# OpenSpaceAI/Nesie

Hardware: AMD Instinct MI355X
Metric: ScanNet scenes/sec (fwd+bwd, 40k pts, bs=8) (higher is better)
Workload: dtype f32; 1 GPU; Nesie-VoteNet supervised pretrain step (nesie-votenet-scannet-pretrain-10%): fwd+bwd+AdamW, 40000 pts/scene, fp32, random-init weights; scenes_per_gpu=8, global_batch=8, parallelism=single, world_size=1, hip_graph=True, deterministic_backward=True, index_chain_pipelined=True, forward_cu_budget=232, forward_cu_budget_from_the_head_on=248, grad_allreduce_bytes=10561936, resident_input_scenes=0

## Files before the change

### include/nesie_ops.h

```cpp
#ifndef NESIE_OPS_H_
#define NESIE_OPS_H_

#include <stddef.h>
#include <stdint.h>

#ifdef __cplusplus
extern "C" {
#endif

typedef enum {
  NESIE_OK = 0,
  NESIE_ERR_INVALID_ARG = 1,
  NESIE_ERR_UNSUPPORTED = 2,
  NESIE_ERR_LAUNCH = 3
} nesie_status;

int nesie_abi_version(void);
const char *nesie_last_error(void);

int nesie_set_distance_form(int form);
int nesie_get_distance_form(void);
int nesie_set_cu_count(int n);
int nesie_get_cu_count(void);

// ... 260 lines not shown

int nesie_pool_tail_pack(int nb, int c, int m, const float *grad_pooled, const float *pooled,
                         const uint8_t *argmax, float *ent, void *stream);
int nesie_pw_dgrad_bn_reduce_sparse(int nb, int ng, int c, int cout, long long p, int ns,
                                    const float *ent, const float *w, long long w_gstride,
                                    int w_rstride, int w_cstride, float *y, long long y_bstride,
                                    const float *bn_z, long long bnz_bstride, const float *bn_coef,
                                    float *bn_part, void *stream);
int nesie_pw_wgrad_sparse_supported(int co, int ci, long long p, int ns);
int nesie_pw_wgrad_sparse(int nb, int ng, int co, int ci, long long p, int ns, const float *ent,
                          const float *x, long long x_bstride, const float *x_coef, float *dw,
                          void *workspace, size_t workspace_bytes, int defer, void *stream);

int nesie_pw_wgrad_supported(int co, int ci, long long p);
int nesie_pw_wgrad_tiled(int nb, int ng, int co, int ci, long long p);
size_t nesie_pw_wgrad_workspace_bytes(int nb, int ng, int co, int ci, long long p);
int nesie_pw_wgrad(int nb, int ng, int co, int ci, long long p, const float *dy,
                   long long dy_bstride, const float *x, long long x_bstride,
                   const float *x_coef, int x_relu, float *dw, void *workspace,
                   size_t workspace_bytes, int defer, void *stream);

int nesie_pw_wgrad_flush_deferred(void *stream);
int nesie_pw_wgrad_pending(void);
int nesie_pw_wgrad_drop_deferred(void);

int nesie_pw_wgrad_bn_supported(int co, int ci, long long p);
int nesie_pw_wgrad_bn_backward(int nb, int ng, int co, int ci, long long p, const float *da,
                               const float *z, long long z_bstride, const float *z_coef,
                               const float *gamma, const float *part, int nslots, const float *x,
                               long long x_bstride, const float *x_coef, int x_relu, float *dz,
                               float *dw, float *dgamma, float *dbeta, float *coef_ws,
                               float *d_row_bias, int rb_group, void *workspace,
                               size_t workspace_bytes, int defer, void *stream);

long long nesie_mlp_stream_partials(int b, long long p);
int nesie_mlp_stat_finalize(int c, long long nparts, double count, const float *stat_partial,
                            const float *gamma, const float *beta, float *running_mean,
                            float *running_var, float momentum, float eps, float *coef,
                            int channel_major, void *stream);
int nesie_mlp_layer_forward_stream(int b, int cin, int cout, long long p, const float *x,
                                   long long x_bstride, const float *w, const float *in_coef,
                                   int in_relu, float *y, float *stat_partial, void *stream);

int nesie_pw_layer_forward_k4(int nb, int cout, long long p, const float *x4, long long x4_bstride,
                              const float *w0, const float *w, int w_rstride, int w_cstride,
                              const float *in_coef, float *y, long long y_bstride, float *stat_part,
                              void *stream);
int nesie_pw_dgrad_bn_reduce_k4(int nb, int k, long long p, const float *x, long long x_bstride,
                                const float *w, int w_rstride, int w_cstride, const float *x4,
                                long long x4_bstride, const float *w0, const float *bn_coef,
                                float *bn_part, float *g_part, void *stream);
int nesie_pw_wgrad_bn_backward_k4(int nb, long long p, const float *da, const float *z,
                                  long long z_bstride, const float *z_coef, const float *gamma,
                                  const float *part, int nslots, const float *x4,
                                  long long x4_bstride, const float *w0, const float *x_coef,
                                  float *dz, float *dw, float *dgamma, float *dbeta, float *coef_ws,
                                  void *workspace, size_t workspace_bytes, int defer, void *stream);
int nesie_pw_wgrad_bn_backward_k4_slots(int nb, long long p);
int nesie_pw_wgrad_bn_backward_k4_fused(int nb, long long p, const float *da, const float *z,
                                        long long z_bstride, const float *z_coef, const float *gamma,
                                        const float *part, int nslots, const float *x4,
                                        long long x4_bstride, const float *w0, const float *x_coef,
                                        const float *w, float *dw, float *dgamma, float *dbeta,
                                        float *coef_ws, float *in_part, float *in_gpart,
                                        void *workspace, size_t workspace_bytes, int defer, void *stream);
size_t nesie_k4_moments_bytes(void);
// ... 23 lines not shown
```

### nesie_amd/csrc/pwconv_wgrad.hip

```cpp
#include "pwconv_fwd.h"

using namespace nesie;

namespace nesie {

template <int CO16, int CI16, int WM, int WN, bool AFF, bool BNB, bool K4 = false, bool FDG = false>
__global__ __launch_bounds__(512, FDG ? 4 : 1) void pw_wgrad_kernel(
    int nb, int ng, int co_all, int ci_all, long long p, const float *__restrict__ dy, long long dy_bs,
    const float *__restrict__ x, long long x_bs, const float *__restrict__ x_coef, int coef_gs,
    float x_lo, float *__restrict__ partial, int nwg_g, const float *__restrict__ bnz,
    const float *__restrict__ bnb, float *dz, float *__restrict__ d_rb, int rb_group, int rev,
    const float *__restrict__ k4_w, const float *__restrict__ fdg_w = nullptr, float *__restrict__ fdg_part = nullptr,
    float *__restrict__ fdg_gpart = nullptr) {
  const int row0 = blockIdx.y * CO16 * 16, col0 = blockIdx.z * CI16 * 16;
  const int co = co_all - row0 < CO16 * 16 ? co_all - row0 : CO16 * 16;
  const int ci = ci_all - col0 < CI16 * 16 ? ci_all - col0 : CI16 * 16;
  dy += (size_t)row0 * p;
  x += (size_t)col0 * p;
  if (AFF) x_coef += (size_t)col0 * 4;
  partial += (size_t)(blockIdx.y * gridDim.z + blockIdx.z) * ng * nwg_g * (CO16 * 16) * (CI16 * 16);
  constexpr int MB = CO16 / WM, NB = CI16 / WN, PT = 32, PITCH = PT + 4, CPR = PT / 4;
  constexpr int ROWS = (CO16 + CI16) * 16, NT = 512;
  constexpr int NX = (ROWS * CPR + NT - 1) / NT;
  constexpr bool EVEN = ROWS * CPR == NX * NT;
  constexpr int DYSLOTS = CO16 * 16 * CPR / NT;
  static_assert(WM * WN == 8 && CO16 % WM == 0 && CI16 % WN == 0 && (CO16 * 16 * CPR) % NT == 0, "tiling");
  extern __shared__ __attribute__((aligned(16))) float lds[];
  constexpr int TILE = ROWS * PITCH + (FDG ? 4 * PITCH : 0);
  static_assert(!FDG || (K4 && BNB && CO16 == 4 && CI16 == 4), "FDG: the 64 x 64 layer over a rebuilt operand");
  const int tid = threadIdx.x, lane = tid & 63, quad = lane >> 4, l16 = lane & 15;
  const int wave = __builtin_amdgcn_readfirstlane(tid >> 6);
  const int wm = wave / WN, wn = wave % WN;
  const int g = blockIdx.x % ng, rank = blockIdx.x / ng;

  static_assert(!K4 || (AFF && NX - DYSLOTS == 1 && CI16 == 4 && EVEN), "K4: one slot of X rows");
  float4 k4w = make_float4(0.f, 0.f, 0.f, 0.f);
  unsigned k4off = 0;
  bool k4row0 = false;
  f32x4 k4x[K4 ? 3 : 1];
  unsigned goff[NX], lw[NX];
  bool okslot[NX];
  float sc[AFF ? NX : 1], bi[AFF ? NX : 1];
  float zsc[BNB ? DYSLOTS : 1], zbi[BNB ? DYSLOTS : 1], za[BNB ? DYSLOTS : 1], zmu[BNB ? DYSLOTS : 1], zd1[BNB ? DYSLOTS : 1], ze0[BNB ? DYSLOTS : 1];
#pragma unroll
  for (int i = 0; i < NX; ++i) {
    const int c = i * NT + tid;
    const int row = c / CPR, cp = c % CPR;
    const bool isdy = i < DYSLOTS;
    const int r = isdy ? row : row - CO16 * 16;
    const bool ok = (EVEN || c < ROWS * CPR) && r < (isdy ? co : ci);
    okslot[i] = ok;
    goff[i] = ok ? (unsigned)(((size_t)r * p + cp * 4) * 4) : 0u;
    lw[i] = (unsigned)((row * PITCH + cp * 4) * 4);
    if constexpr (K4) {
      if (!isdy) {
        k4w = *(const float4 *)(k4_w + (size_t)r * 4);
        k4off = (unsigned)(cp * 16);
        k4row0 = r == 0;
        asm volatile("" : "+v"(k4w.x), "+v"(k4w.y), "+v"(k4w.z), "+v"(k4w.w));
      }
    }
    if (AFF) {
// ... 33 lines not shown
    const float *dyb = dy + pend, *xb = x + (size_t)n * x_bs + p0;
#pragma unroll
    for (int i = 0; i < NX; ++i) {
      unsigned o = goff[i];
      asm volatile("" : "+v"(o));
      if constexpr (K4) {
        if (i >= DYSLOTS) {
          unsigned o4 = k4off;
          asm volatile("" : "+v"(o4));
          stg[i] = load16_saddr(o4, xb);
#pragma unroll
          for (int j = 1; j < 4; ++j) k4x[j - 1] = load16_saddr(o4, xb + (size_t)j * p);
          continue;
        }
      }
      stg[i] = load16_saddr(o, i < DYSLOTS ? dyb : xb);
      if constexpr (BNB) {
        if (i < DYSLOTS) stz[i] = load16_saddr(o, bnz + pend);
      }
    }
  };
  auto write_tile = [&](float *buf) {
#pragma unroll
    for (int i = 0; i < NX; ++i) {
      f32x4 q = stg[i];
      if constexpr (BNB) {
        if (i < DYSLOTS) {
#pragma unroll
          for (int e = 0; e < 4; ++e) {
            const float zz = stz[i][e];
            const float gg = __builtin_fmaf(zz, zsc[i], zbi[i]) > 0.f ? q[e] : 0.f;
            q[e] = __builtin_fmaf(za[i], gg, __builtin_fmaf(zmu[i] - zz, zd1[i], ze0[i]));
          }
          if constexpr (!FDG) {
            if (pend_ok && okslot[i]) *(f32x4 *)((char *)(dz + pend) + goff[i]) = q;
          }
          if (d_rb) {
            float tsum = (q[0] + q[1]) + (q[2] + q[3]);
            tsum += __shfl_xor(tsum, 1, 64);
            tsum += __shfl_xor(tsum, 2, 64);
            if (rb_group == 64) tsum += __shfl_xor(tsum, 4, 64);
            const int c_ = i * NT + tid, row = c_ / CPR, cp = c_ % CPR;
            const bool writer = rb_group == 64 ? cp == 0 : (cp & 3) == 0;
            if (pend_ok && okslot[i] && writer) {
              const int gsh = rb_group == 64 ? 6 : 4;
              float *dst = d_rb + ((size_t)pend_n * co + row) * (size_t)(p >> gsh) + ((pend_p0 + 4 * cp) >> gsh);
              if (rb_group == 64) atomicAdd(dst, tsum); else *dst = tsum;
            }
          }
        }
      }
      if constexpr (K4) {
        if (i >= DYSLOTS) {
          if constexpr (FDG) {
            if (k4row0) {
              float *xt = buf + ROWS * PITCH + (k4off >> 2);
              *(f32x4 *)(xt) = q;
              *(f32x4 *)(xt + PITCH) = k4x[0];
              *(f32x4 *)(xt + 2 * PITCH) = k4x[1];
              *(f32x4 *)(xt + 3 * PITCH) = k4x[2];
            }
          }
#pragma unroll
          for (int e = 0; e < 4; ++e) q[e] = k4_dot(k4w, q[e], k4x[0][e], k4x[1][e], k4x[2][e]);
        }
      }
      if (AFF && i >= DYSLOTS) {
#pragma unroll
        for (int e = 0; e < 4; ++e) q[e] = fmaxf(__builtin_fmaf(q[e], sc[i], bi[i]), x_lo);
      }
      if (!(EVEN && all_rows)) q = okslot[i] ? q : (f32x4){0.f, 0.f, 0.f, 0.f};
      if (EVEN || (i * NT + tid) < ROWS * CPR) *(f32x4 *)((char *)buf + lw[i]) = q;
    }
  };

  f32x4 acc[MB][NB];
#pragma unroll
  for (int i = 0; i < MB; ++i)
#pragma unroll
    for (int j = 0; j < NB; ++j) acc[i][j] = (f32x4){0.f, 0.f, 0.f, 0.f};
  const int cb = wave & 3, ph = wave >> 2;
  float fw[FDG ? 16 : 1];
  float4 fw0 = make_float4(0.f, 0.f, 0.f, 0.f), fco = fw0;
  float fr0 = 0.f, fr1 = 0.f, fgx[4] = {0.f, 0.f, 0.f, 0.f};
  if constexpr (FDG) {
    const int c = 16 * cb + l16;
#pragma unroll
    for (int kk = 0; kk < 16; ++kk) fw[kk] = fdg_w[(size_t)(4 * kk + quad) * 64 + c];
    fw0 = *(const float4 *)(k4_w + (size_t)c * 4);
    fco = *(const float4 *)(x_coef + (size_t)c * 4);
#pragma unroll
    for (int kk = 0; kk < 16; ++kk) asm volatile("" : "+v"(fw[kk]));
    asm volatile("" : "+v"(fw0.x), "+v"(fw0.y), "+v"(fw0.z), "+v"(fw0.w), "+v"(fco.x), "+v"(fco.y), "+v"(fco.z), "+v"(fco.w));
  }

  float *b0 = lds, *b1 = lds + TILE;
  int t = rank;
  if (t < ntiles) {
    load_tile(t);
    write_tile(b0);
    load_tile(t + nwg_g);
  }
  for (; t < ntiles; t += nwg_g) {
    lgkm_wait<0>();
    __builtin_amdgcn_s_barrier();
    const unsigned la = lds_addr(b0) + (unsigned)(((wm * MB * 16 + l16) * PITCH + 4 * quad) * 4);
    const unsigned lb = lds_addr(b0) + (unsigned)(((CO16 * 16 + wn * NB * 16 + l16) * PITCH + 4 * quad) * 4);
    f32x4 fa[MB], fb[NB];
    static_for<0, 2>([&](auto pgc) {
      constexpr int pg = decltype(pgc)::value;
      static_for<0, MB>([&](auto ic) {
        constexpr int i = decltype(ic)::value;
        fa[i] = lds_read_b128<(i * 16 * PITCH + 16 * pg) * 4>(la);
      });
      static_for<0, NB>([&](auto jc) {
        constexpr int j = decltype(jc)::value;
        fb[j] = lds_read_b128<(j * 16 * PITCH + 16 * pg) * 4>(lb);
      });
      lgkm_wait<0>();
      __builtin_amdgcn_sched_barrier(0);
      static_for<0, 4>([&](auto cc) {
        constexpr int c = decltype(cc)::value;
        static_for<0, MB>([&](auto ic) {
          constexpr int i = decltype(ic)::value;
          static_for<0, NB>([&](auto jc) {
            constexpr int j = decltype(jc)::value;
            acc[i][j] = __builtin_amdgcn_mfma_f32_16x16x4f32(fa[i][c], fb[j][c], acc[i][j], 0, 0, 0);
          });
        });
      });
      __builtin_amdgcn_sched_barrier(0);
    });
    if constexpr (FDG) {
      f32x4 da = {0.f, 0.f, 0.f, 0.f};
      const float *az = b0 + quad * PITCH + 16 * ph + l16;
#pragma unroll
      for (int kk = 0; kk < 16; ++kk)
        da = __builtin_amdgcn_mfma_f32_16x16x4f32(az[kk * 4 * PITCH], fw[kk], da, 0, 0, 0);
      const float *xt = b0 + ROWS * PITCH + 16 * ph + 4 * quad;
      const f32x4 x0 = *(const f32x4 *)xt, x1 = *(const f32x4 *)(xt + PITCH), x2 = *(const f32x4 *)(xt + 2 * PITCH),
                  x3 = *(const f32x4 *)(xt + 3 * PITCH);
#pragma unroll
      for (int r = 0; r < 4; ++r) {
        const float z = k4_dot(fw0, x0[r], x1[r], x2[r], x3[r]);
        const float gg = __builtin_fmaf(z, fco.x, fco.y) > 0.f ? da[r] : 0.f;
        fr0 += gg;
        fr1 += gg * ((z - fco.z) * fco.w);
        fgx[0] = __builtin_fmaf(gg, x0[r], fgx[0]);
        fgx[1] = __builtin_fmaf(gg, x1[r], fgx[1]);
        fgx[2] = __builtin_fmaf(gg, x2[r], fgx[2]);
        fgx[3] = __builtin_fmaf(gg, x3[r], fgx[3]);
      }
    }
    write_tile(b1);
    __builtin_amdgcn_sched_barrier(0);
    load_tile(t + 2 * nwg_g);
    float *const tb = b0; b0 = b1; b1 = tb;
  }
  if constexpr (FDG) {
    float v[6] = {fr0, fr1, fgx[0], fgx[1], fgx[2], fgx[3]};
#pragma unroll
    for (int u = 0; u < 6; ++u) {
      v[u] += __shfl_xor(v[u], 16, 64);
      v[u] += __shfl_xor(v[u], 32, 64);
    }
    if (quad == 0) {
      const int c = 16 * cb + l16, slot = 2 * rank + ph, nslots = 2 * nwg_g;
      *(float2 *)(fdg_part + ((size_t)c * nslots + slot) * 2) = make_float2(v[0], v[1]);
      *(float4 *)(fdg_gpart + ((size_t)c * nslots + slot) * 4) = make_float4(v[2], v[3], v[4], v[5]);
    }
  }
  const bool tiled = gridDim.y * gridDim.z > 1;
  float *dst = partial + ((size_t)g * nwg_g + rank) * (tiled ? (size_t)(CO16 * 16) * (CI16 * 16) : (size_t)co * ci);
#pragma unroll
  for (int i = 0; i < MB; ++i)
#pragma unroll
    for (int j = 0; j < NB; ++j)
#pragma unroll
      for (int r = 0; r < 4; ++r) {
        const int m = (wm * MB + i) * 16 + 4 * quad + r, k = (wn * NB + j) * 16 + l16;
        if (m < co && k < ci) dst[(size_t)m * ci + k] = acc[i][j][r];
      }
}

__global__ __launch_bounds__(512) void pw_wgrad_sparse_kernel(int nb, int ng, long long p, const float *__restrict__ x,
                                                              long long x_bs, const float *__restrict__ coef,
                                                              const float2 *__restrict__ ent, int ns_shift,
                                                              int groups, float *__restrict__ partial, int nwg,
// ... 249 lines not shown
constexpr int TILED_B = 64, TILED_MAX_TILES = 1024;
static bool pw_wgrad_tiled(int nb, int ng, int co, int ci, long long p) {
  if (nb <= 0 || ng <= 0 || nb % ng || p <= 0 || p % 32 || ci < 9 || ci > 1024 || co < 1 || co > 1024) return false;
  const long long tiles = (long long)(nb / ng) * (p / 32);
  return tiles <= TILED_MAX_TILES && (long long)co * ci >= 128 * 192;
}
static int pw_wgrad_tiled_nwg(int nb, int ng, int co, int ci, long long p) {
  const long long tiles = (long long)(nb / ng) * (p / 32);
  const int blocks = cdiv(co, TILED_B) * cdiv(ci, TILED_B);
  long long nwg = 512 / ((long long)blocks * ng);
  if (nwg < 1) nwg = 1;
  if (nwg > tiles) nwg = tiles;
  return (int)nwg;
}

extern "C" int nesie_pw_wgrad_tiled(int nb, int ng, int co, int ci, long long p) {
  return pw_wgrad_tiled(nb, ng, co, ci, p) ? 1 : 0;
}

extern "C" size_t nesie_pw_wgrad_workspace_bytes(int nb, int ng, int co, int ci, long long p) {
  if (nb <= 0 || ng <= 0 || p <= 0) return 0;
  const size_t whole = (size_t)ng * pw_wgrad_nwg(nb, ng, p, co, pw_wgrad_block(co, ci)) * co * pw_wgrad_block(co, ci) * sizeof(float);
  const size_t tiled = (size_t)cdiv(co, TILED_B) * cdiv(ci, TILED_B) * ng * pw_wgrad_tiled_nwg(nb, ng, co, ci, p) *
                       TILED_B * TILED_B * sizeof(float);
  return whole > tiled ? whole : tiled;
}

namespace nesie {
__global__ __launch_bounds__(64) void pw_bnb_coef_kernel(int channels, int nslots, double count,
                                                         const float *__restrict__ part,
                                                         const float *__restrict__ z_coef,
                                                         const float *__restrict__ gamma,
                                                         float *__restrict__ bnb, float *__restrict__ dgamma,
                                                         float *__restrict__ dbeta) {
  const int c = blockIdx.x;
  double s0 = 0.0, s1 = 0.0;
  const float2 *pc = (const float2 *)part + (size_t)c * nslots;
  int i = threadIdx.x;
  for (; i + 192 < nslots; i += 256) {
    float2 q[4];
#pragma unroll
    for (int u = 0; u < 4; ++u) q[u] = pc[i + 64 * u];
#pragma unroll
    for (int u = 0; u < 4; ++u) { s0 += (double)q[u].x; s1 += (double)q[u].y; }
  }
  for (; i < nslots; i += 64) {
    const float2 q = pc[i];
    s0 += (double)q.x;
    s1 += (double)q.y;
  }
#pragma unroll
  for (int off = 32; off > 0; off >>= 1) {
    s0 += __shfl_xor(s0, off, 64);
    s1 += __shfl_xor(s1, off, 64);
  }
  if (threadIdx.x == 0) {
    const float invstd = z_coef[c * 4 + 3];
    const float a = (float)((gamma ? (double)gamma[c] : 1.0) * (double)invstd);
    const float k1 = (float)(s0 / count), k2 = (float)(s1 / count);
    float *o = bnb + (size_t)c * 8;
    o[0] = z_coef[c * 4 + 0]; o[1] = z_coef[c * 4 + 1]; o[2] = a; o[3] = z_coef[c * 4 + 2];
    o[4] = a * invstd * k2; o[5] = -a * k1; o[6] = 0.f; o[7] = 0.f;
    if (dbeta) dbeta[c] = (float)s0;
    if (dgamma) dgamma[c] = (float)s1;
  }
}

struct PwWgrad {
  int nb, ng, co, ci; long long p;
  const float *dy; long long dy_bs;
  const float *x; long long x_bs;
  const float *x_coef; int x_relu;
  float *dw; void *workspace; size_t workspace_bytes;
  int defer;
  const float *bnz, *bnb; float *dz;
  float *d_rb; int rb_group;
  const float *k4_w;
  const float *fdg_w; float *fdg_part, *fdg_gpart;
  const float *sp_ent; int sp_ns;
  const float *z_coef, *gamma, *part; int nslots;
  float *dgamma, *dbeta, *coef_ws;
};

constexpr size_t pw_wgrad_lds(int co16, int ci16, bool fdg = false) {
  return (size_t)2 * ((co16 + ci16) * 16 * 36 + (fdg ? 4 * 36 : 0)) * sizeof(float);
}

template <auto Kern, typename... Args>
static void launch_lds(dim3 grid, size_t lds, hipStream_t s, Args... args) {
  static bool attr = false;
  if (!attr) {
    (void)hipFuncSetAttribute((const void *)Kern, hipFuncAttributeMaxDynamicSharedMemorySize, (int)lds);
    attr = true;
  }
  hipLaunchKernelGGL(Kern, grid, dim3(512), lds, s, args...);
}

static int rd_defer(const RDesc &d, hipStream_t s) {
  if (g_pending.n == RD_MAX) { const int st = rd_flush(s); if (st) return st; }
  rd_push(d);
  return NESIE_OK;
}

static int pw_wgrad_launch(const char *W, const PwWgrad &d, hipStream_t s) {
  const int nb = d.nb, ng = d.ng, co = d.co, ci = d.ci;
  const long long p = d.p;
  NESIE_REQUIRE(nb >= 0 && ng >= 1 && co >= 1 && ci >= 1 && p >= 0 && d.dw, W);
  NESIE_REQUIRE(!d.sp_ent || (co == 128 && ci == 256 && (d.sp_ns == 16 || d.sp_ns == 64) && p % d.sp_ns == 0 && d.x_coef &&
                              d.x_relu && !d.bnb && !d.d_rb && !d.k4_w && ((uintptr_t)d.sp_ent & 7) == 0), W);
  NESIE_REQUIRE(!d.k4_w || (co == 64 && ci == 64 && ng == 1 && d.bnb && d.x_coef && !d.d_rb && d.x_bs >= 4 * p &&
                            ((uintptr_t)d.k4_w & 15) == 0), W);
  if (nb == 0 || p == 0) {
    (void)hipMemsetAsync(d.dw, 0, (size_t)ng * co * ci * sizeof(float), s);
    return NESIE_OK;
  }
  const bool tiled_mode = !d.bnb && !d.d_rb && pw_wgrad_tiled(nb, ng, co, ci, p);
  if (!tiled_mode && !nesie_pw_wgrad_supported(co, ci, p)) {
    set_error("%s: %d x %d over %lld positions is outside the built tiles", W, co, ci, p);
    return NESIE_ERR_UNSUPPORTED;
  }
  NESIE_REQUIRE(nb % ng == 0 && (d.dy || d.sp_ent) && d.x && d.workspace, W);
  NESIE_REQUIRE(d.workspace_bytes >= nesie_pw_wgrad_workspace_bytes(nb, ng, co, ci, p), W);
  NESIE_REQUIRE((((uintptr_t)d.dy | (uintptr_t)d.x) & 15) == 0 && (d.dy_bs & 3) == 0 && (d.x_bs & 3) == 0, W);
  NESIE_REQUIRE((long long)(co > ci ? co : ci) * p < (1ll << 30), W);
  NESIE_REQUIRE((long long)(nb / ng) * (p / 32) < (1ll << 30), W);
  const float lo = d.x_relu ? 0.f : -__builtin_inff();
  const int rev = walk_dir((long long)nb * co * p * 4);
  float *partial = (float *)d.workspace;
  int nwg = 0, cw = 0;
  dim3 grid;
  const float *xc = nullptr, *cc = nullptr;
  auto launch_sparse = [&](int tiled) {
    launch_lds<pw_wgrad_sparse_kernel>(dim3(nwg * ng), (size_t)2 * 256 * 36 * sizeof(float) + 256 * sizeof(float2), s, nb,
                                       ng, p, d.x, d.x_bs, d.x_coef, (const float2 *)d.sp_ent, d.sp_ns == 16 ? 4 : 6,
                                       (int)(p / d.sp_ns), partial, nwg, rev, tiled);
  };
#define LKL(LDS, ...)                                                                                                  \
  launch_lds<pw_wgrad_kernel<__VA_ARGS__>>(grid, LDS, s, nb, ng, co, cw, p, d.dy, d.dy_bs, xc, d.x_bs, cc, ci, lo,     \
                                           partial, nwg, d.bnz, d.bnb, d.dz, d.d_rb, d.rb_group, rev, d.k4_w, d.fdg_w, \
                                           d.fdg_part, d.fdg_gpart)
#define LK(CO16, CI16, ...) LKL(pw_wgrad_lds(CO16, CI16), CO16, CI16, __VA_ARGS__)
  if (tiled_mode) {
    nwg = pw_wgrad_tiled_nwg(nb, ng, co, ci, p);
    const int nrb = cdiv(co, TILED_B), ncb = cdiv(ci, TILED_B);
    grid = dim3(nwg * ng, nrb, ncb);
    cw = ci; xc = d.x; cc = d.x_coef;
    if (d.sp_ent) launch_sparse(1);
    else if (d.x_coef) LK(4, 4, 2, 4, true, false); else LK(4, 4, 2, 4, false, false);
    if (d.defer) {
      RDesc r{};
      r.part = partial; r.dw = d.dw; r.kind = 1; r.nparts = nwg; r.ci = ci; r.co = co; r.ng = ng;
      r.br = TILED_B; r.bc = TILED_B; r.nblk = nrb * ncb;
      const int st = rd_defer(r, s);
      return st ? st : check_launch(W);
    }
    hipLaunchKernelGGL(pw_wgrad_reduce_tiled_kernel, dim3(cdiv(TILED_B * TILED_B, 256), nrb * ncb, ng), dim3(256), 0, s,
                       co, ci, TILED_B, TILED_B, nwg, partial, d.dw);
    return check_launch(W);
  }
  const int block = pw_wgrad_block(co, ci);
  NESIE_REQUIRE(!d.bnb || (d.bnz && d.dz && block == ci && (((uintptr_t)d.bnz | (uintptr_t)d.dz) & 15) == 0), W);
  NESIE_REQUIRE(!d.d_rb || (d.bnb && (d.rb_group == 16 || d.rb_group == 64) && p % d.rb_group == 0 &&
                            d.dy_bs == (long long)co * p), W);
  nwg = pw_wgrad_nwg(nb, ng, p, co, block, d.bnb != nullptr);
  grid = dim3(nwg * ng);
#define L(CO16, CI16, WM, WN)                                                                                          \
  do {                                                                                                                 \
    if (d.bnb) { if (d.x_coef) LK(CO16, CI16, WM, WN, true, true); else LK(CO16, CI16, WM, WN, false, true); }         \
    else { if (d.x_coef) LK(CO16, CI16, WM, WN, true, false); else LK(CO16, CI16, WM, WN, false, false); }             \
  } while (0)
  for (int c0 = 0; c0 < ci; c0 += block) {
    cw = ci - c0 < block ? ci - c0 : block;
    xc = d.x + (size_t)c0 * p;
    cc = d.x_coef ? d.x_coef + (size_t)c0 * 4 : nullptr;
    if (d.k4_w && d.fdg_w) {
      NESIE_REQUIRE(d.fdg_part && d.fdg_gpart && ((uintptr_t)d.fdg_gpart & 15) == 0 && ((uintptr_t)d.fdg_part & 7) == 0, W);
      LKL(pw_wgrad_lds(4, 4, true), 4, 4, 2, 4, true, true, true, true);
    } else if (d.k4_w) LK(4, 4, 2, 4, true, true, true);
    else if (d.sp_ent) launch_sparse(0);
    else if (co <= 64 && cw <= 64) L(4, 4, 2, 4);
    else if (co <= 128 && cw <= 64) L(8, 4, 4, 2);
    else if (co <= 128 && cw <= 128) L(8, 8, 2, 4);
    else if (co <= 128 && cw <= 192) L(8, 12, 2, 4);
    else if (co <= 128 && cw <= 256) L(8, 16, 2, 4);
    else if (co <= 128) L(8, 20, 2, 4);
    else L(16, 8, 4, 2);
    const int total = co * cw;
    if (d.defer && block >= ci) {
      RDesc r{};
      r.part = partial; r.dw = d.dw; r.kind = 0; r.nparts = nwg; r.total = total; r.ci = cw; r.ld = ci; r.col0 = c0;
      r.co = co; r.ng = ng;
      const int st = rd_defer(r, s);
      if (st) return st;
      continue;
    }
    hipLaunchKernelGGL(pw_wgrad_reduce_kernel, dim3(cdiv(total, 64), ng), dim3(1024), 0, s, total, nwg,
                       partial, d.dw, cw, ci, c0, co);
  }
#undef L
#undef LK
#undef LKL
  return check_launch(W);
}

static PwWgrad pw_wgrad_problem(int nb, int ng, int co, int ci, long long p, float *dw, void *workspace,
                                size_t workspace_bytes) {
  PwWgrad d{};
  d.nb = nb; d.ng = ng; d.co = co; d.ci = ci; d.p = p;
  d.dw = dw; d.workspace = workspace; d.workspace_bytes = workspace_bytes;
  return d;
}
// ... 17 lines not shown
extern "C" int nesie_pw_wgrad_sparse(int nb, int ng, int co, int ci, long long p, int ns, const float *ent,
                                     const float *x, long long x_bstride, const float *x_coef, float *dw,
                                     void *workspace, size_t workspace_bytes, int defer, void *stream) {
  const char *W = "pw_wgrad_sparse";
  NESIE_REQUIRE(ent && nesie_pw_wgrad_sparse_supported(co, ci, p, ns), W);
  PwWgrad d = pw_wgrad_problem(nb, ng, co, ci, p, dw, workspace, workspace_bytes);
  d.x = x; d.x_bs = x_bstride; d.x_coef = x_coef; d.x_relu = 1;
  d.sp_ent = ent; d.sp_ns = ns;
  d.defer = defer;
  return pw_wgrad_launch(W, d, (hipStream_t)stream);
}

extern "C" int nesie_pw_wgrad_flush_deferred(void *stream) { return rd_flush((hipStream_t)stream); }
extern "C" int nesie_pw_wgrad_pending(void) { return g_pending.n; }
extern "C" int nesie_pw_wgrad_drop_deferred(void) {
  g_pending.n = 0;
  return NESIE_OK;
}

extern "C" int nesie_pw_wgrad_bn_supported(int co, int ci, long long p) {
  return nesie_pw_wgrad_supported(co, ci, p) && pw_wgrad_block(co, ci) == ci ? 1 : 0;
}

static int pw_wgrad_bn_backward_impl(const char *W, PwWgrad d, void *stream) {
  const int nb = d.nb, ng = d.ng, co = d.co;
  NESIE_REQUIRE(nb >= 0 && ng >= 1 && co >= 1 && d.nslots >= 1, W);
  hipStream_t s = (hipStream_t)stream;
  if (nb == 0 || d.p == 0) {
    if (d.dgamma) (void)hipMemsetAsync(d.dgamma, 0, (size_t)ng * co * sizeof(float), s);
    if (d.dbeta) (void)hipMemsetAsync(d.dbeta, 0, (size_t)ng * co * sizeof(float), s);
    return pw_wgrad_launch(W, d, s);
  }
  NESIE_REQUIRE(d.dy && d.bnz && d.z_coef && d.part && d.dz && d.coef_ws && nb % ng == 0, W);
  hipLaunchKernelGGL(pw_bnb_coef_kernel, dim3(ng * co), dim3(64), 0, s, ng * co, d.nslots,
                     (double)(nb / ng) * (double)d.p, d.part, d.z_coef, d.gamma, d.coef_ws, d.dgamma, d.dbeta);
  d.bnb = d.coef_ws;
  return pw_wgrad_launch(W, d, s);
}

extern "C" int nesie_pw_wgrad_bn_backward(int nb, int ng, int co, int ci, long long p, const float *da,
                                          const float *z, long long z_bstride, const float *z_coef,
                                          const float *gamma, const float *part, int nslots,
                                          const float *x, long long x_bstride, const float *x_coef,
                                          int x_relu, float *dz, float *dw, float *dgamma, float *dbeta,
                                          float *coef_ws, float *d_row_bias, int rb_group,
                                          void *workspace, size_t workspace_bytes, int defer, void *stream) {
  PwWgrad d = pw_wgrad_problem(nb, ng, co, ci, p, dw, workspace, workspace_bytes);
  d.dy = da; d.bnz = z; d.dy_bs = z_bstride; d.dz = dz;
  d.z_coef = z_coef; d.gamma = gamma; d.part = part; d.nslots = nslots;
  d.x = x; d.x_bs = x_bstride; d.x_coef = x_coef; d.x_relu = x_relu;
  d.dgamma = dgamma; d.dbeta = dbeta; d.coef_ws = coef_ws;
  d.d_rb = d_row_bias; d.rb_group = rb_group;
  d.defer = defer;
  return pw_wgrad_bn_backward_impl("pw_wgrad_bn_backward", d, stream);
}

extern "C" int nesie_pw_wgrad_bn_backward_k4(int nb, long long p, const float *da, const float *z,
                                             long long z_bstride, const float *z_coef, const float *gamma,
                                             const float *part, int nslots, const float *x4,
                                             long long x4_bstride, const float *w0, const float *x_coef,
                                             float *dz, float *dw, float *dgamma, float *dbeta, float *coef_ws,
                                             void *workspace, size_t workspace_bytes, int defer, void *stream) {
  const char *W = "pw_wgrad_bn_backward_k4";
  NESIE_REQUIRE(nb >= 1 && p >= 32 && x4 && w0 && x_coef, W);
  PwWgrad d = pw_wgrad_problem(nb, 1, 64, 64, p, dw, workspace, workspace_bytes);
  d.dy = da; d.bnz = z; d.dy_bs = z_bstride; d.dz = dz;
  d.z_coef = z_coef; d.gamma = gamma; d.part = part; d.nslots = nslots;
  d.x = x4; d.x_bs = x4_bstride; d.x_coef = x_coef; d.x_relu = 1; d.k4_w = w0;
  d.dgamma = dgamma; d.dbeta = dbeta; d.coef_ws = coef_ws;
  d.defer = defer;
  return pw_wgrad_bn_backward_impl(W, d, stream);
}

extern "C" int nesie_pw_wgrad_bn_backward_k4_slots(int nb, long long p) {
  return 2 * pw_wgrad_nwg(nb, 1, p, 64, 64, true);
}
extern "C" int nesie_pw_wgrad_bn_backward_k4_fused(int nb, long long p, const float *da, const float *z,
                                                   long long z_bstride, const float *z_coef, const float *gamma,
                                                   const float *part, int nslots, const float *x4,
                                                   long long x4_bstride, const float *w0, const float *x_coef,
                                                   const float *w, float *dw, float *dgamma, float *dbeta,
                                                   float *coef_ws, float *in_part, float *in_gpart,
                                                   void *workspace, size_t workspace_bytes, int defer,
                                                   void *stream) {
  const char *W = "pw_wgrad_bn_backward_k4_fused";
  NESIE_REQUIRE(nb >= 1 && p >= 32 && x4 && w0 && x_coef && w && in_part && in_gpart, W);
  PwWgrad d = pw_wgrad_problem(nb, 1, 64, 64, p, dw, workspace, workspace_bytes);
  d.dy = da; d.bnz = z; d.dy_bs = z_bstride; d.dz = const_cast<float *>(da);
  d.z_coef = z_coef; d.gamma = gamma; d.part = part; d.nslots = nslots;
  d.x = x4; d.x_bs = x4_bstride; d.x_coef = x_coef; d.x_relu = 1; d.k4_w = w0;
  d.fdg_w = w; d.fdg_part = in_part; d.fdg_gpart = in_gpart;
  d.dgamma = dgamma; d.dbeta = dbeta; d.coef_ws = coef_ws;
  d.defer = defer;
  return pw_wgrad_bn_backward_impl(W, d, stream);
}

extern "C" int nesie_pw_bnb_coef(int channels, int nslots, double count, const float *part,
                                 const float *z_coef, const float *gamma, float *bnb, float *dgamma,
                                 float *dbeta, void *stream) {
  const char *W = "pw_bnb_coef";
  NESIE_REQUIRE(channels >= 0 && nslots >= 1 && count > 0, W);
  if (channels == 0) return NESIE_OK;
  NESIE_REQUIRE(part && z_coef && bnb, W);
  hipLaunchKernelGGL(pw_bnb_coef_kernel, dim3(channels), dim3(64), 0, (hipStream_t)stream, channels, nslots,
                     count, part, z_coef, gamma, bnb, dgamma, dbeta);
  return check_launch(W);
}
```

### nesie_amd/kernels.py

```python
import contextlib
import os

import ctypes

import torch

from . import _lib

_injected = None


def _no_cpu_path(device):
    return RuntimeError(
        "nesie_amd kernels need HIP device tensors (got device "
        f"{device}); there is no CPU path in the product")


def _check(*tensors):
    for t in tensors:
        if not t.is_cuda:
            raise _no_cpu_path(t.device)
        if not t.is_contiguous():
            raise RuntimeError("nesie_amd kernels need contiguous tensors")

# ... 618 lines not shown
        if defer:
            HipKernels._deferred.append((ws, dw))
        return ws, need, defer

    def pw_wgrad(self, dy, x, dw, ng=1, x_coef=None, x_relu=True, final=False):
        _f32(dy, x, dw)
        nb, co, p = dy.shape
        ci = x.shape[1]
        assert dy.is_cuda and x.shape[0] == nb and x.shape[2] == p and nb % ng == 0
        assert dw.is_contiguous() and dw.numel() == ng * co * ci
        assert x.stride(2) == 1 and x.stride(1) == p and dy.stride(2) == 1 and dy.stride(1) == p
        if x_coef is not None:
            _check(x_coef); _f32(x_coef)
            assert tuple(x_coef.shape) == (ng * ci, 4)
        ws, need, defer = self._wgrad_scratch(nb, ng, co, ci, p, dw, final)
        _launch("nesie_pw_wgrad", dy, nb, ng, co, ci, p, dy, dy.stride(0) if nb > 1 else co * p, x,
                x.stride(0) if nb > 1 else ci * p, x_coef, bool(x_relu), dw, ws, need, defer)

    def pw_bnb_coef(self, part, z_coef, gamma, count, dgamma, dbeta):
        _check(part, z_coef, dgamma, dbeta); _f32(part, z_coef, dgamma, dbeta)
        ch = part.shape[0]
        assert part.dim() == 3 and part.shape[2] == 2 and tuple(z_coef.shape) == (ch, 4)
        assert dgamma.numel() == ch == dbeta.numel()
        if gamma is not None:
            _check(gamma); _f32(gamma)
        bnb = torch.empty(ch, 8, dtype=torch.float32, device=part.device)
        _launch("nesie_pw_bnb_coef", part, ch, part.shape[1], float(count), part, z_coef, gamma,
                bnb, dgamma, dbeta)
        return bnb

    def pw_wgrad_bn_supported(self, co, ci, p):
        return bool(_lib.load().nesie_pw_wgrad_bn_supported(int(co), int(ci), int(p)))

    def pw_wgrad_bn_backward(self, da, z, z_coef, gamma, part, x, dz, dw, dgamma, dbeta, ng=1,
                             x_coef=None, x_relu=True, d_row_bias=None, group=0, final=False):
        _f32(da, z, x, dz, dw, dgamma, dbeta); _check(z_coef, part, dz); _f32(z_coef, part)
        nb, co, p = da.shape
        ci = x.shape[1]
        assert da.is_cuda and tuple(z.shape) == (nb, co, p) == tuple(dz.shape) and x.shape[0] == nb
        assert x.shape[2] == p and nb % ng == 0 and da.is_contiguous() and z.is_contiguous()
        assert dw.is_contiguous() and dw.numel() == ng * co * ci
        assert x.stride(2) == 1 and x.stride(1) == p
        assert tuple(z_coef.shape) == (ng * co, 4) and part.dim() == 3 and part.shape[0] == ng * co
        assert dgamma.numel() == ng * co == dbeta.numel()
        if d_row_bias is not None:
            _check(d_row_bias); _f32(d_row_bias)
            assert group in (16, 64) and d_row_bias.numel() == nb * co * (p // group)
        if gamma is not None:
            _check(gamma); _f32(gamma)
        if x_coef is not None:
            _check(x_coef); _f32(x_coef)
            assert tuple(x_coef.shape) == (ng * ci, 4)
        ws, need, defer = self._wgrad_scratch(nb, ng, co, ci, p, dw, final)
        cws = torch.empty(ng * co, 8, dtype=torch.float32, device=da.device)
        _launch("nesie_pw_wgrad_bn_backward", da, nb, ng, co, ci, p, da, z, co * p, z_coef, gamma,
                part, part.shape[1], x, x.stride(0) if nb > 1 else ci * p, x_coef, bool(x_relu), dz,
                dw, dgamma, dbeta, cws, d_row_bias, int(group), ws, need, defer)

    @staticmethod
    def conv_wgrad_supported(cout, cin):
        return (cout <= 128 and cin <= 288) or (cout <= 256 and cin <= 128)

    @staticmethod
    def _bn_pool_ws(x):
        b, c, m, ns = x.shape
        need = _lib.load().nesie_bn_workspace_bytes(b, c, m * ns)
        return _workspace(need, x.device), need

    def bn_relu_maxpool_forward(self, x, gamma, beta, running_mean, running_var, momentum, eps,
                                pooled, argmax, save_mean, save_invstd, fwd_coef):
        _check(x, pooled, argmax, save_mean, save_invstd, fwd_coef); _f32(x, pooled)
        b, c, m, ns = x.shape
        assert tuple(pooled.shape) == (b, c, m) and argmax.dtype == torch.uint8
        ws, need = self._bn_pool_ws(x)
        _launch("nesie_bn_relu_maxpool_forward", x, b, c, m, ns, x, gamma, beta, running_mean,
                running_var, float(momentum), float(eps), pooled, argmax, save_mean, save_invstd,
                fwd_coef, ws, need)

    def bn_relu_maxpool_backward(self, grad_pooled, argmax, x, pooled, gamma, save_invstd,
                                 fwd_coef, dx, dgamma, dbeta):
        _check(grad_pooled, argmax, x, pooled, dx); _f32(grad_pooled, x, pooled, dx)
        b, c, m, ns = x.shape
        assert tuple(grad_pooled.shape) == (b, c, m) and dx.shape == x.shape
        ws, need = self._bn_pool_ws(x)
        _launch("nesie_bn_relu_maxpool_backward", x, b, c, m, ns, grad_pooled, argmax, x, pooled,
                gamma, save_invstd, fwd_coef, dx, dgamma, dbeta, ws, need)

# ... 519 lines not shown
```

### nesie_amd/mmdet3d_ops/fused_mlp.py

```python

import torch
from torch.autograd import Function

from .. import grad_slots
from ..kernels import backend_for


ENABLED = True
SA1_K4 = True
FOLD_NORM_BWD = True

_OWNED_MARK = '_nesie_fresh_grad'


def _dst(slot, like, *shape):
    return slot.view(*shape) if slot is not None else like.new_empty(*shape)


def _into(slot, g):
    if slot is None or g is None:
        return g
    slot.view(g.shape).copy_(g)
    return slot.view(g.shape)

# ... 539 lines not shown
        ctx.G = G
        ctx.slots = [grad_slots.take(t) if ctx.needs_input_grad[5 + j] else None
                     for j, t in enumerate((gamma1, beta1, w4))]
        ctx.save_for_backward(c, y, coef1, arg, wl, gamma1, beta1, w4)
        ctx.mark_non_differentiable(arg)
        return out

    @staticmethod
    def backward(ctx, dout):
        c, y, coef1, arg, wl, gamma1, beta1, w4 = ctx.saved_tensors
        backend = backend_for(c)
        B, S, half, P = c.shape
        H2, F = wl.shape[1], w4.shape[1]
        G = ctx.G
        yf = y.view(B * S, H2, P)
        dw4 = None
        da = c.new_empty(B * S, H2, P)
        if mini_tail_sparse_supported(backend, F, H2, G, P):
            ent = backend.pool_tail_pack(dout.contiguous().view(B * S, F, P // G), arg.view(B * S, F, P // G))
            if ctx.needs_input_grad[7]:
                dw4 = _dst(ctx.slots[2], c, S, F, H2)
                backend.pw_wgrad_sparse(ent, G, yf, dw4, ng=S, x_coef=coef1, final=ctx.slots[2] is not None)
            part = backend.pw_dgrad_bn_reduce_sparse(ent, G, w4.transpose(1, 2), yf, coef1, da, ng=S)
        else:
            dz = c.new_empty(B, S, F, P // G, G)
            backend.group_max_pool_backward(dout.contiguous(), arg, dz)
            dzf = dz.view(B * S, F, P)
            if ctx.needs_input_grad[7]:
                dw4 = _wgrad(backend, dzf, yf, coef1, ng=S, slot=ctx.slots[2])
            part = backend.pw_dgrad_bn_reduce(dzf, w4.transpose(1, 2), yf, coef1, da, ng=S)
        dgamma, dbeta = _dst(ctx.slots[0], c, S * H2), _dst(ctx.slots[1], c, S * H2)
        cf = c.view(B * S, half, P)
        dwl = None
        if (FOLD_NORM_BWD and ctx.needs_input_grad[4] and G in (16, 64)
                and backend.pw_wgrad_bn_supported(H2, half, P)):
            dsmall = (c.new_zeros if G == 64 else c.new_empty)(B, S, H2, P // G)
            dwl = c.new_empty(S, H2, half)
            backend.pw_wgrad_bn_backward(da, yf, coef1, gamma1, part, cf, da, dwl, dgamma, dbeta, ng=S,
                                         x_coef=None, d_row_bias=dsmall.view(B * S, H2, -1), group=G)
            dyf = da
        else:
            dy = torch.empty_like(y)
            dsmall = c.new_empty(B, S, H2, P // G)
            backend.bn_relu_backward_apply(da.view(B, S * H2, P), y.view(B, S * H2, P), gamma1,
                                           None, coef1, part, dy.view(B, S * H2, P), dgamma, dbeta,
                                           d_row_bias=dsmall.view(B, S * H2, -1), group=G)
            dyf = dy.view(B * S, H2, P)
            if ctx.needs_input_grad[4]:
                dwl = _wgrad(backend, dyf, cf, None, ng=S)
        dc = torch.empty_like(c)
        backend.pw_layer_forward(dyf, wl.transpose(1, 2), ng=S, y=dc.view(B * S, half, P))
        setattr(dc, _OWNED_MARK, True)
        return dc, dsmall, None, None, dwl, dgamma, dbeta, dw4


MINI_TAIL_SPARSE = True


def mini_tail_sparse_supported(backend, F, H2, G, P):
    return (MINI_TAIL_SPARSE and backend.name == 'hip' and F == 128 and H2 == 256 and G in (16, 64)
            and P % 64 == 0 and backend.pw_wgrad_sparse_supported(F, H2, P, G))


def mini_pointnets_fused_supported(backend, c0, c0_part, G):
    if not ENABLED or backend.name != 'hip' or c0.dtype != torch.float32 or c0_part is None \
            or G not in (16, 64):
        return False
    B, S, H0, P = c0.shape[0], c0.shape[1], c0.shape[2], c0.shape[3] * c0.shape[4]
    return (c0_part.numel() > 0 and backend.pw_supported(H0, H0 // 2, P)
            and backend.pw_supported(H0 // 2, H0, P))



class SplitXyzFeat(Function):

    @staticmethod
    def forward(ctx, w):
        S, H, K = w.shape
        ctx.dims = (S, H, K)
        ctx.slot = grad_slots.take(w) if ctx.needs_input_grad[0] else None
        return w[:, :, :3].contiguous(), w[:, :, 3:].reshape(S * H, K - 3)

    @staticmethod
    def backward(ctx, d_xyz, d_feat):
        S, H, K = ctx.dims
        like = d_xyz if d_xyz is not None else d_feat
        if d_xyz is None:
            d_xyz = like.new_zeros(S, H, 3)
        if d_feat is None:
# ... 224 lines not shown
```

Measured before the change: 686.6 scenes/s.

## Fuse input-gradient GEMM into BN-folded weight-gradient kernel for 256x128 mini-tail layer

Adds a DG variant of the BN-backward weight-gradient kernel that reuses the dy tile already staged in LDS to compute the input gradient dx = W^T·dy with extra MFMA ops, writing dx directly. The weight is rearranged into an MFMA-friendly layout inside the BN coefficient kernel. This removes the separate pw_layer_forward dgrad launch and the write and reread of the dz activation buffer. The cost is more registers and per-tile work in the wgrad loop, which may lengthen its critical path.

Result: no change. 690.3 scenes/s, median of 6 (+0.5%).

```diff
diff --git a/include/nesie_ops.h b/include/nesie_ops.h
--- a/include/nesie_ops.h
+++ b/include/nesie_ops.h
@@ -316,6 +316,14 @@
                                float *dw, float *dgamma, float *dbeta, float *coef_ws,
                                float *d_row_bias, int rb_group, void *workspace,
                                size_t workspace_bytes, int defer, void *stream);
+int nesie_pw_wgrad_bn_dgrad_supported(int co, int ci, long long p);
+int nesie_pw_wgrad_bn_backward_dgrad(int nb, int ng, int co, int ci, long long p, const float *da,
+                                     const float *z, long long z_bstride, const float *z_coef,
+                                     const float *gamma, const float *part, int nslots, const float *x,
+                                     long long x_bstride, const float *w, float *dx, float *dw,
+                                     float *dgamma, float *dbeta, float *coef_ws, float *d_row_bias,
+                                     int rb_group, void *workspace, size_t workspace_bytes, int defer,
+                                     void *stream);
 
 long long nesie_mlp_stream_partials(int b, long long p);
 int nesie_mlp_stat_finalize(int c, long long nparts, double count, const float *stat_partial,
diff --git a/nesie_amd/csrc/pwconv_wgrad.hip b/nesie_amd/csrc/pwconv_wgrad.hip
--- a/nesie_amd/csrc/pwconv_wgrad.hip
+++ b/nesie_amd/csrc/pwconv_wgrad.hip
@@ -4,14 +4,22 @@
 
 namespace nesie {
 
-template <int CO16, int CI16, int WM, int WN, bool AFF, bool BNB, bool K4 = false, bool FDG = false>
+template <int OFF>
+__device__ __forceinline__ f32x2 lds_read_b64(unsigned addr) {
+  static_assert(OFF >= 0 && OFF < 65536, "ds_read_b64 reach");
+  f32x2 v;
+  asm volatile("ds_read_b64 %0, %1 offset:%2" : "=v"(v) : "v"(addr), "n"(OFF));
+  return v;
+}
+
+template <int CO16, int CI16, int WM, int WN, bool AFF, bool BNB, bool K4 = false, bool FDG = false, bool DG = false>
 __global__ __launch_bounds__(512, FDG ? 4 : 1) void pw_wgrad_kernel(
     int nb, int ng, int co_all, int ci_all, long long p, const float *__restrict__ dy, long long dy_bs,
     const float *__restrict__ x, long long x_bs, const float *__restrict__ x_coef, int coef_gs,
     float x_lo, float *__restrict__ partial, int nwg_g, const float *__restrict__ bnz,
     const float *__restrict__ bnb, float *dz, float *__restrict__ d_rb, int rb_group, int rev,
     const float *__restrict__ k4_w, const float *__restrict__ fdg_w = nullptr, float *__restrict__ fdg_part = nullptr,
-    float *__restrict__ fdg_gpart = nullptr) {
+    float *__restrict__ fdg_gpart = nullptr, const float *__restrict__ dg_w = nullptr, float *__restrict__ dg_dx = nullptr) {
   const int row0 = blockIdx.y * CO16 * 16, col0 = blockIdx.z * CI16 * 16;
   const int co = co_all - row0 < CO16 * 16 ? co_all - row0 : CO16 * 16;
   const int ci = ci_all - col0 < CI16 * 16 ? ci_all - col0 : CI16 * 16;
@@ -28,6 +36,7 @@
   extern __shared__ __attribute__((aligned(16))) float lds[];
   constexpr int TILE = ROWS * PITCH + (FDG ? 4 * PITCH : 0);
   static_assert(!FDG || (K4 && BNB && CO16 == 4 && CI16 == 4), "FDG: the 64 x 64 layer over a rebuilt operand");
+  static_assert(!DG || (BNB && !K4 && !FDG && CO16 == 16 && CI16 == 8), "DG: the 256 x 128 layer");
   const int tid = threadIdx.x, lane = tid & 63, quad = lane >> 4, l16 = lane & 15;
   const int wave = __builtin_amdgcn_readfirstlane(tid >> 6);
   const int wm = wave / WN, wn = wave % WN;
@@ -127,7 +136,7 @@
             const float gg = __builtin_fmaf(zz, zsc[i], zbi[i]) > 0.f ? q[e] : 0.f;
             q[e] = __builtin_fmaf(za[i], gg, __builtin_fmaf(zmu[i] - zz, zd1[i], ze0[i]));
           }
-          if constexpr (!FDG) {
+          if constexpr (!FDG && !DG) {
             if (pend_ok && okslot[i]) *(f32x4 *)((char *)(dz + pend) + goff[i]) = q;
           }
           if (d_rb) {
@@ -189,16 +198,34 @@
     asm volatile("" : "+v"(fw0.x), "+v"(fw0.y), "+v"(fw0.z), "+v"(fw0.w), "+v"(fco.x), "+v"(fco.y), "+v"(fco.z), "+v"(fco.w));
   }
 
+  constexpr int DGK = CO16 * 4, DGC = DGK / 4, DGR = 8, DGA = 4;
+  f32x4 dgr[DG ? DGR : 1];
+  const float *dgw_g = DG ? dg_w + ((size_t)g * 8 + wave) * (DGC * 256) : nullptr;
+  const unsigned dgw_off = (unsigned)(lane * 16);
+  const unsigned dgx_off = (unsigned)(((size_t)(16 * wave + l16) * p + 8 * quad) * 4);
+  int cur_n = 0, cur_p0 = 0;
+  auto dg_load = [&](auto jc) {
+    constexpr int j = decltype(jc)::value;
+    unsigned o = dgw_off;
+    asm volatile("" : "+v"(o));
+    dgr[j % DGR] = load16_saddr(o, dgw_g + j * 256);
+  };
+
   float *b0 = lds, *b1 = lds + TILE;
   int t = rank;
   if (t < ntiles) {
     load_tile(t);
     write_tile(b0);
+    cur_n = pend_n; cur_p0 = pend_p0;
     load_tile(t + nwg_g);
   }
   for (; t < ntiles; t += nwg_g) {
     lgkm_wait<0>();
     __builtin_amdgcn_s_barrier();
+    if constexpr (DG) {
+      static_for<0, DGA>([&](auto jc) { dg_load(jc); });
+      __builtin_amdgcn_sched_barrier(0);
+    }
     const unsigned la = lds_addr(b0) + (unsigned)(((wm * MB * 16 + l16) * PITCH + 4 * quad) * 4);
     const unsigned lb = lds_addr(b0) + (unsigned)(((CO16 * 16 + wn * NB * 16 + l16) * PITCH + 4 * quad) * 4);
     f32x4 fa[MB], fb[NB];
@@ -247,8 +274,44 @@
         fgx[3] = __builtin_fmaf(gg, x3[r], fgx[3]);
       }
     }
+    f32x4 dgacc[DG ? 2 : 1];
+    if constexpr (DG) {
+      static_assert(DGK == 64 && 2 * DGA <= DGR && (DGK * 4 * PITCH * 4) < 65536, "DG: 64 steps over 256 rows");
+      const unsigned az = lds_addr(b0) + (unsigned)((quad * PITCH + 2 * l16) * 4);
+      dgacc[0] = dgacc[1] = (f32x4){0.f, 0.f, 0.f, 0.f};
+      constexpr int PF = 2;
+      f32x2 fr[PF + 1];
+      auto read_frag = [&](auto kkc) {
+        constexpr int kk = decltype(kkc)::value;
+        fr[kk % (PF + 1)] = lds_read_b64<kk * 4 * PITCH * 4>(az);
+      };
+      static_for<0, PF>([&](auto kkc) { read_frag(kkc); });
+      static_for<0, DGK>([&](auto kkc) {
+        constexpr int kk = decltype(kkc)::value;
+        if constexpr (kk + PF < DGK) {
+          read_frag(std::integral_constant<int, kk + PF>{});
+          lgkm_wait<PF>();
+        } else {
+          lgkm_wait<(DGK - 1 - kk)>();
+        }
+        __builtin_amdgcn_sched_barrier(0);
+        dgacc[0] = __builtin_amdgcn_mfma_f32_16x16x4f32(fr[kk % (PF + 1)][0], dgr[(kk / 4) % DGR][kk % 4], dgacc[0], 0, 0, 0);
+        dgacc[1] = __builtin_amdgcn_mfma_f32_16x16x4f32(fr[kk % (PF + 1)][1], dgr[(kk / 4) % DGR][kk % 4], dgacc[1], 0, 0, 0);
+        __builtin_amdgcn_sched_barrier(0);
+        if constexpr (kk % 4 == 3 && kk / 4 + DGA < DGC) {
+          dg_load(std::integral_constant<int, kk / 4 + DGA>{});
+          __builtin_amdgcn_sched_barrier(0);
+        }
+      });
+    }
     write_tile(b1);
     __builtin_amdgcn_sched_barrier(0);
+    if constexpr (DG) {
+      float *xt = dg_dx + (size_t)cur_n * (CI16 * 16) * p + cur_p0;
+      store16_saddr<0>(dgx_off, (f32x4){dgacc[0][0], dgacc[1][0], dgacc[0][1], dgacc[1][1]}, xt);
+      store16_saddr<16>(dgx_off, (f32x4){dgacc[0][2], dgacc[1][2], dgacc[0][3], dgacc[1][3]}, xt);
+      cur_n = pend_n; cur_p0 = pend_p0;
+    }
     load_tile(t + 2 * nwg_g);
     float *const tb = b0; b0 = b1; b1 = tb;
   }
@@ -564,8 +627,16 @@
                                                          const float *__restrict__ z_coef,
                                                          const float *__restrict__ gamma,
                                                          float *__restrict__ bnb, float *__restrict__ dgamma,
-                                                         float *__restrict__ dbeta) {
+                                                         float *__restrict__ dbeta,
+                                                         const float *__restrict__ w_src = nullptr,
+                                                         float *__restrict__ w_dst = nullptr) {
   const int c = blockIdx.x;
+  if (w_src) {
+    const int g = c >> 8, r = c & 255;
+    for (int cc = threadIdx.x; cc < 128; cc += 64)
+      w_dst[((((size_t)g * 8 + (cc >> 4)) * 16 + (r >> 4)) * 64 + (r & 3) * 16 + (cc & 15)) * 4 + ((r >> 2) & 3)] =
+          w_src[(size_t)c * 128 + cc];
+  }
   double s0 = 0.0, s1 = 0.0;
   const float2 *pc = (const float2 *)part + (size_t)c * nslots;
   int i = threadIdx.x;
@@ -609,6 +680,7 @@
   float *d_rb; int rb_group;
   const float *k4_w;
   const float *fdg_w; float *fdg_part, *fdg_gpart;
+  const float *dg_w; float *dg_dx;
   const float *sp_ent; int sp_ns;
   const float *z_coef, *gamma, *part; int nslots;
   float *dgamma, *dbeta, *coef_ws;
@@ -670,7 +742,7 @@
 #define LKL(LDS, ...)                                                                                                  \
   launch_lds<pw_wgrad_kernel<__VA_ARGS__>>(grid, LDS, s, nb, ng, co, cw, p, d.dy, d.dy_bs, xc, d.x_bs, cc, ci, lo,     \
                                            partial, nwg, d.bnz, d.bnb, d.dz, d.d_rb, d.rb_group, rev, d.k4_w, d.fdg_w, \
-                                           d.fdg_part, d.fdg_gpart)
+                                           d.fdg_part, d.fdg_gpart, d.dg_w, d.dg_dx)
 #define LK(CO16, CI16, ...) LKL(pw_wgrad_lds(CO16, CI16), CO16, CI16, __VA_ARGS__)
   if (tiled_mode) {
     nwg = pw_wgrad_tiled_nwg(nb, ng, co, ci, p);
@@ -709,6 +781,11 @@
       NESIE_REQUIRE(d.fdg_part && d.fdg_gpart && ((uintptr_t)d.fdg_gpart & 15) == 0 && ((uintptr_t)d.fdg_part & 7) == 0, W);
       LKL(pw_wgrad_lds(4, 4, true), 4, 4, 2, 4, true, true, true, true);
     } else if (d.k4_w) LK(4, 4, 2, 4, true, true, true);
+    else if (d.dg_w) {
+      NESIE_REQUIRE(co == 256 && cw == 128 && d.bnb && !d.x_coef && !d.sp_ent && d.dg_dx && p % 64 == 0 &&
+                    (((uintptr_t)d.dg_w | (uintptr_t)d.dg_dx) & 15) == 0, W);
+      LK(16, 8, 4, 2, false, true, false, false, true);
+    }
     else if (d.sp_ent) launch_sparse(0);
     else if (co <= 64 && cw <= 64) L(4, 4, 2, 4);
     else if (co <= 128 && cw <= 64) L(8, 4, 4, 2);
@@ -792,8 +869,11 @@
     return pw_wgrad_launch(W, d, s);
   }
   NESIE_REQUIRE(d.dy && d.bnz && d.z_coef && d.part && d.dz && d.coef_ws && nb % ng == 0, W);
+  float *const wp = d.dg_w ? d.coef_ws + (size_t)ng * co * 8 : nullptr;
   hipLaunchKernelGGL(pw_bnb_coef_kernel, dim3(ng * co), dim3(64), 0, s, ng * co, d.nslots,
-                     (double)(nb / ng) * (double)d.p, d.part, d.z_coef, d.gamma, d.coef_ws, d.dgamma, d.dbeta);
+                     (double)(nb / ng) * (double)d.p, d.part, d.z_coef, d.gamma, d.coef_ws, d.dgamma, d.dbeta,
+                     d.dg_w, wp);
+  if (wp) d.dg_w = wp;
   d.bnb = d.coef_ws;
   return pw_wgrad_launch(W, d, s);
 }
@@ -855,6 +935,31 @@
   return pw_wgrad_bn_backward_impl(W, d, stream);
 }
 
+extern "C" int nesie_pw_wgrad_bn_dgrad_supported(int co, int ci, long long p) {
+  return co == 256 && ci == 128 && p > 0 && p % 64 == 0 && (long long)co * p < (1ll << 30) &&
+                 nesie_pw_wgrad_bn_supported(co, ci, p) ? 1 : 0;
+}
+extern "C" int nesie_pw_wgrad_bn_backward_dgrad(int nb, int ng, int co, int ci, long long p, const float *da,
+                                                const float *z, long long z_bstride, const float *z_coef,
+                                                const float *gamma, const float *part, int nslots,
+                                                const float *x, long long x_bstride, const float *w, float *dx,
+                                                float *dw, float *dgamma, float *dbeta, float *coef_ws,
+                                                float *d_row_bias, int rb_group, void *workspace,
+                                                size_t workspace_bytes, int defer, void *stream) {
+  const char *W = "pw_wgrad_bn_backward_dgrad";
+  NESIE_REQUIRE(nb >= 0 && ng >= 1 && nesie_pw_wgrad_bn_dgrad_supported(co, ci, p) && w && dx &&
+                z_bstride == (long long)co * p, W);
+  PwWgrad d = pw_wgrad_problem(nb, ng, co, ci, p, dw, workspace, workspace_bytes);
+  d.dy = da; d.bnz = z; d.dy_bs = z_bstride; d.dz = const_cast<float *>(da);
+  d.z_coef = z_coef; d.gamma = gamma; d.part = part; d.nslots = nslots;
+  d.x = x; d.x_bs = x_bstride; d.x_relu = 0;
+  d.dg_w = w; d.dg_dx = dx;
+  d.dgamma = dgamma; d.dbeta = dbeta; d.coef_ws = coef_ws;
+  d.d_rb = d_row_bias; d.rb_group = rb_group;
+  d.defer = defer;
+  return pw_wgrad_bn_backward_impl(W, d, stream);
+}
+
 extern "C" int nesie_pw_bnb_coef(int channels, int nslots, double count, const float *part,
                                  const float *z_coef, const float *gamma, float *bnb, float *dgamma,
                                  float *dbeta, void *stream) {
@@ -863,6 +968,6 @@
   if (channels == 0) return NESIE_OK;
   NESIE_REQUIRE(part && z_coef && bnb, W);
   hipLaunchKernelGGL(pw_bnb_coef_kernel, dim3(channels), dim3(64), 0, (hipStream_t)stream, channels, nslots,
-                     count, part, z_coef, gamma, bnb, dgamma, dbeta);
+                     count, part, z_coef, gamma, bnb, dgamma, dbeta, (const float *)nullptr, (float *)nullptr);
   return check_launch(W);
 }
diff --git a/nesie_amd/kernels.py b/nesie_amd/kernels.py
--- a/nesie_amd/kernels.py
+++ b/nesie_amd/kernels.py
@@ -674,8 +674,20 @@
     def pw_wgrad_bn_supported(self, co, ci, p):
         return bool(_lib.load().nesie_pw_wgrad_bn_supported(int(co), int(ci), int(p)))
 
+    def pw_wgrad_bn_dgrad_supported(self, co, ci, p):
+        return bool(_lib.load().nesie_pw_wgrad_bn_dgrad_supported(int(co), int(ci), int(p)))
+
     def pw_wgrad_bn_backward(self, da, z, z_coef, gamma, part, x, dz, dw, dgamma, dbeta, ng=1,
-                             x_coef=None, x_relu=True, d_row_bias=None, group=0, final=False):
+                             x_coef=None, x_relu=True, d_row_bias=None, group=0, final=False,
+                             dgrad_w=None, dgrad_out=None):
+        fused = dgrad_w is not None or dgrad_out is not None
+        if fused:
+            if dgrad_w is None or dgrad_out is None:
+                raise ValueError("pw_wgrad_bn_backward: dgrad_w and dgrad_out come together")
+            if dz is not None or x_coef is not None:
+                raise ValueError("pw_wgrad_bn_backward: the fused input gradient writes no dz and takes a plain x")
+            _check(dgrad_w, dgrad_out); _f32(dgrad_w, dgrad_out)
+            dz = da
         _f32(da, z, x, dz, dw, dgamma, dbeta); _check(z_coef, part, dz); _f32(z_coef, part)
         nb, co, p = da.shape
         ci = x.shape[1]
@@ -693,8 +705,17 @@
         if x_coef is not None:
             _check(x_coef); _f32(x_coef)
             assert tuple(x_coef.shape) == (ng * ci, 4)
+        if fused:
+            if not self.pw_wgrad_bn_dgrad_supported(co, ci, p):
+                raise RuntimeError(f"pw_wgrad_bn_backward: no fused input gradient at {co} x {ci} over {p} positions")
+            assert tuple(dgrad_w.shape) == (ng, co, ci) and tuple(dgrad_out.shape) == (nb, ci, p)
         ws, need, defer = self._wgrad_scratch(nb, ng, co, ci, p, dw, final)
-        cws = torch.empty(ng * co, 8, dtype=torch.float32, device=da.device)
+        cws = torch.empty(ng * co, 8 + (ci if fused else 0), dtype=torch.float32, device=da.device)
+        if fused:
+            _launch("nesie_pw_wgrad_bn_backward_dgrad", da, nb, ng, co, ci, p, da, z, co * p, z_coef, gamma,
+                    part, part.shape[1], x, x.stride(0) if nb > 1 else ci * p, dgrad_w, dgrad_out, dw,
+                    dgamma, dbeta, cws, d_row_bias, int(group), ws, need, defer)
+            return
         _launch("nesie_pw_wgrad_bn_backward", da, nb, ng, co, ci, p, da, z, co * p, z_coef, gamma,
                 part, part.shape[1], x, x.stride(0) if nb > 1 else ci * p, x_coef, bool(x_relu), dz,
                 dw, dgamma, dbeta, cws, d_row_bias, int(group), ws, need, defer)
diff --git a/nesie_amd/mmdet3d_ops/fused_mlp.py b/nesie_amd/mmdet3d_ops/fused_mlp.py
--- a/nesie_amd/mmdet3d_ops/fused_mlp.py
+++ b/nesie_amd/mmdet3d_ops/fused_mlp.py
@@ -595,13 +595,20 @@
         dgamma, dbeta = _dst(ctx.slots[0], c, S * H2), _dst(ctx.slots[1], c, S * H2)
         cf = c.view(B * S, half, P)
         dwl = None
+        dc = torch.empty_like(c)
+        dyf = None
         if (FOLD_NORM_BWD and ctx.needs_input_grad[4] and G in (16, 64)
                 and backend.pw_wgrad_bn_supported(H2, half, P)):
             dsmall = (c.new_zeros if G == 64 else c.new_empty)(B, S, H2, P // G)
             dwl = c.new_empty(S, H2, half)
-            backend.pw_wgrad_bn_backward(da, yf, coef1, gamma1, part, cf, da, dwl, dgamma, dbeta, ng=S,
-                                         x_coef=None, d_row_bias=dsmall.view(B * S, H2, -1), group=G)
-            dyf = da
+            if mini_tail_dgrad_fused_supported(backend, H2, half, P):
+                backend.pw_wgrad_bn_backward(da, yf, coef1, gamma1, part, cf, None, dwl, dgamma, dbeta, ng=S,
+                                             x_coef=None, d_row_bias=dsmall.view(B * S, H2, -1), group=G,
+                                             dgrad_w=wl.contiguous(), dgrad_out=dc.view(B * S, half, P))
+            else:
+                backend.pw_wgrad_bn_backward(da, yf, coef1, gamma1, part, cf, da, dwl, dgamma, dbeta, ng=S,
+                                             x_coef=None, d_row_bias=dsmall.view(B * S, H2, -1), group=G)
+                dyf = da
         else:
             dy = torch.empty_like(y)
             dsmall = c.new_empty(B, S, H2, P // G)
@@ -611,13 +618,19 @@
             dyf = dy.view(B * S, H2, P)
             if ctx.needs_input_grad[4]:
                 dwl = _wgrad(backend, dyf, cf, None, ng=S)
-        dc = torch.empty_like(c)
-        backend.pw_layer_forward(dyf, wl.transpose(1, 2), ng=S, y=dc.view(B * S, half, P))
+        if dyf is not None:
+            backend.pw_layer_forward(dyf, wl.transpose(1, 2), ng=S, y=dc.view(B * S, half, P))
         setattr(dc, _OWNED_MARK, True)
         return dc, dsmall, None, None, dwl, dgamma, dbeta, dw4
 
 
 MINI_TAIL_SPARSE = True
+MINI_TAIL_DGRAD_FUSED = True
+
+
+def mini_tail_dgrad_fused_supported(backend, H2, half, P):
+    return (MINI_TAIL_DGRAD_FUSED and backend.name == 'hip'
+            and backend.pw_wgrad_bn_dgrad_supported(H2, half, P))
 
 
 def mini_tail_sparse_supported(backend, F, H2, G, P):
```
